# HueCodes/sudoku-vision

Hardware: AMD Instinct MI355X
Metric: end-to-end frames/sec (1080p->81 digits) (higher is better)
Workload: dtype f32

## Files before the change

sudoku-vision_amd/csrc/k1_threshold.hip:

```cpp
#include "sv_device.h"
#include "sv_internal.h"
#include "k2_cells_body.h"

namespace {

constexpr int TW = 64, TH = 32;
constexpr int GW = TW + 14, GH = TH + 14;
constexpr int BW = TW + 10, BH = TH + 10;

struct Taps11 { float k[11]; };

__global__ __launch_bounds__(256) void k_preprocess_any(const u8 *__restrict__ bgr, int H, int W, ptrdiff_t pitch,
                                                          ptrdiff_t img_stride, u8 *__restrict__ out, Taps11 taps)
{
    __shared__ u8 g[GH][GW + 2];
    __shared__ unsigned short hb[GH][BW + 2];
    __shared__ float bl[BH][BW + 1];
    __shared__ float rw[BH][TW + 1];

    const int tid = threadIdx.x;
    const int x0 = blockIdx.x * TW, y0 = blockIdx.y * TH;
    const u8 *img = bgr + (ptrdiff_t)blockIdx.z * img_stride;
    u8 *dst = out + (ptrdiff_t)blockIdx.z * H * W;

    for (int i = tid; i < GH * GW; i += 256) {
        const int ly = i / GW, lx = i - ly * GW;
        const int sx = sv_reflect101(sv_clamp(x0 - 7 + lx, -2, W + 1), W);
        const int sy = sv_reflect101(sv_clamp(y0 - 7 + ly, -2, H + 1), H);
        const u8 *p = img + (ptrdiff_t)sy * pitch + (ptrdiff_t)sx * 3;
        g[ly][lx] = (u8)sv_gray_px(p[0], p[1], p[2]);
    }
    __syncthreads();

    for (int i = tid; i < GH * BW; i += 256) {
        const int ly = i / BW, bq = i - ly * BW;
        const int lc = sv_clamp(x0 - 5 + bq, 0, W - 1) - (x0 - 7);
        hb[ly][bq] = (unsigned short)(16 * (g[ly][lc - 2] + g[ly][lc + 2]) + 64 * (g[ly][lc - 1] + g[ly][lc + 1]) +
                                      96 * g[ly][lc]);
    }
    __syncthreads();

    for (int i = tid; i < BH * BW; i += 256) {
        const int br = i / BW, bq = i - br * BW;
        const int lr = sv_clamp(y0 - 5 + br, 0, H - 1) - (y0 - 7);
        const unsigned v = 16u * (hb[lr - 2][bq] + hb[lr + 2][bq]) + 64u * (hb[lr - 1][bq] + hb[lr + 1][bq]) + 96u * hb[lr][bq];
        bl[br][bq] = (float)((v + 32768u) >> 16);
    }
    __syncthreads();

    for (int i = tid; i < BH * TW; i += 256) {
        const int br = i / TW, x = i - br * TW;
        float acc = __fmul_rn(taps.k[0], bl[br][x]);
#pragma unroll
        for (int j = 1; j < 11; j++) acc = __builtin_fmaf(bl[br][x + j], taps.k[j], acc);
        rw[br][x] = acc;
    }
    __syncthreads();

    for (int i = tid; i < TH * TW; i += 256) {
        const int y = i / TW, x = i - y * TW;
        if (x0 + x >= W || y0 + y >= H) continue;
        float acc = __fmul_rn(taps.k[5], rw[y + 5][x]);
#pragma unroll
        for (int j = 1; j <= 5; j++) acc = __builtin_fmaf(__fadd_rn(rw[y + 5 + j][x], rw[y + 5 - j][x]), taps.k[5 + j], acc);
        const int mean = sv_clamp(__float2int_rn(acc), 0, 255);
        const int src = (int)bl[y + 5][x + 5];
        dst[(ptrdiff_t)(y0 + y) * W + (x0 + x)] = (src - mean <= -2) ? 255 : 0;
    }
}


typedef unsigned int u32;
struct __attribute__((packed, aligned(4))) u32x3 { u32 a, b, c; };
typedef float f32x4_t __attribute__((ext_vector_type(4)));

__device__ __forceinline__ float lane_prev(float v)
{
    return __int_as_float(__builtin_amdgcn_update_dpp(0, __float_as_int(v), 0x138 , 0xf, 0xf, true));
}
__device__ __forceinline__ float lane_next(float v)
{
    return __int_as_float(__builtin_amdgcn_update_dpp(0, __float_as_int(v), 0x130 , 0xf, 0xf, true));
}
__device__ __forceinline__ u32 lane_next_u32(u32 v) { return __float_as_uint(lane_next(__uint_as_float(v))); }
__device__ __forceinline__ float add_prev(float a, float b)
{
    float r;
    asm("v_add_f32_dpp %0, %1, %2 wave_shr:1 row_mask:0xf bank_mask:0xf bound_ctrl:0" : "=v"(r) : "v"(a), "v"(b));
    return r;
}
__device__ __forceinline__ float add_next(float a, float b)
{
    float r;
    asm("v_add_f32_dpp %0, %1, %2 wave_shl:1 row_mask:0xf bank_mask:0xf bound_ctrl:0" : "=v"(r) : "v"(a), "v"(b));
    return r;
}

__device__ __forceinline__ float gray_f32(float b, float g, float r)
{
    return floorf(__builtin_fmaf(b, 3735.f / 32768.f, __builtin_fmaf(g, 19235.f / 32768.f, __builtin_fmaf(r, 9798.f / 32768.f, 0.5f))));
}
__device__ __forceinline__ float blur5(float a, float b, float c, float d, float e)
{
    return __builtin_fmaf(6.f, c, __builtin_fmaf(4.f, b + d, a + e));
}

template <int TW, int TH, int NT, int RC, int RE>
__global__ __launch_bounds__(NT) void k_preprocess_f32(const u8 *__restrict__ bgr, int H, int W, ptrdiff_t pitch,
                                                       ptrdiff_t img_stride, u8 *__restrict__ out, Taps11 taps, int aligned4)
{
    constexpr int GW = TW + 16, GH = TH + 14, BH = TH + 10, NG = GW / 4, NK = TW / 4, NWAVE = NT / 64;
    constexpr int ROWS_PER_WAVE = 64 / NG;
    static_assert(BH * TW <= GH * GW, "rw must fit in hf");
    __shared__ __attribute__((aligned(16))) float smem[GH * GW + BH * GW];
    f32x4_t *hf4 = (f32x4_t *)smem;
    f32x4_t *rw4 = (f32x4_t *)smem;
    f32x4_t *bf4 = (f32x4_t *)(smem + GH * GW);
    float *bf = smem + GH * GW;

    const int tid = threadIdx.x, lane = tid & 63, wave = tid >> 6;
    const int x0 = blockIdx.x * TW, y0 = blockIdx.y * TH;
    const u8 *img = bgr + (ptrdiff_t)blockIdx.z * img_stride;
    u8 *dst = out + (ptrdiff_t)blockIdx.z * H * W;

    {
        const int rl = lane / NG, g = lane - rl * NG;
        const int gx = x0 - 8 + 4 * g;
        const bool fast = aligned4 && gx >= 0 && gx + 3 < W;
        for (int base = 0; base < GH; base += NWAVE * ROWS_PER_WAVE) {
            const int ly = base + wave * ROWS_PER_WAVE + rl;
            const int lyc = ly < GH ? ly : GH - 1;
            const int sy = sv_reflect101(sv_clamp(y0 - 7 + lyc, -2, H + 1), H);
            const u8 *row = img + (ptrdiff_t)sy * pitch;
            float p0, p1, p2, p3;
            if (fast) {
                const u32x3 d = *(const u32x3 *)(row + 3 * gx);
                p0 = gray_f32((float)(d.a & 255), (float)((d.a >> 8) & 255), (float)((d.a >> 16) & 255));
                p1 = gray_f32((float)(d.a >> 24), (float)(d.b & 255), (float)((d.b >> 8) & 255));
                p2 = gray_f32((float)((d.b >> 16) & 255), (float)(d.b >> 24), (float)(d.c & 255));
                p3 = gray_f32((float)((d.c >> 8) & 255), (float)((d.c >> 16) & 255), (float)(d.c >> 24));
            } else {
                float q[4];
                for (int i = 0; i < 4; i++) {
                    const int sx = sv_reflect101(sv_clamp(gx + i, -2, W + 1), W);
                    const u8 *p = row + (ptrdiff_t)sx * 3;
                    q[i] = gray_f32((float)p[0], (float)p[1], (float)p[2]);
                }
                p0 = q[0]; p1 = q[1]; p2 = q[2]; p3 = q[3];
            }
            const float l2 = lane_prev(p2), l3 = lane_prev(p3), r0 = lane_next(p0), r1 = lane_next(p1);
            f32x4_t h;
            h[0] = blur5(l2, l3, p0, p1, p2);
            h[1] = blur5(l3, p0, p1, p2, p3);
            h[2] = blur5(p0, p1, p2, p3, r0);
            h[3] = blur5(p1, p2, p3, r0, r1);
            if (lane < ROWS_PER_WAVE * NG && ly < GH) hf4[ly * NG + g] = h;
        }
    }
    __syncthreads();

    {
        constexpr int NCH = (BH + RC - 1) / RC;
        for (int it = tid; it < NCH * NG; it += NT) {
            const int ch = it / NG, g = it - ch * NG;
            const int br0 = ch * RC;
            f32x4_t win[RC + 4];
#pragma unroll
            for (int r = 0; r < RC + 4; r++) win[r] = hf4[(br0 + r < GH ? br0 + r : GH - 1) * NG + g];
#pragma unroll
            for (int r = 0; r < RC; r++) {
                if (br0 + r < BH) {
                    f32x4_t o;
#pragma unroll
                    for (int c = 0; c < 4; c++)
                        o[c] = floorf(__builtin_fmaf(blur5(win[r][c], win[r + 1][c], win[r + 2][c], win[r + 3][c], win[r + 4][c]), 1.f / 256.f, 0.5f));
                    bf4[(br0 + r) * NG + g] = o;
                }
            }
        }
    }
    __syncthreads();

    if (x0 < 5 || x0 + TW + 5 > W || y0 < 5 || y0 + TH + 5 > H) {
        for (int it = tid; it < BH * GW; it += NT) {
            const int br = it / GW, c = it - br * GW;
            const int q = x0 - 8 + c;
            if (q < 0 || q >= W) {
                const int sc = sv_clamp(q, 0, W - 1) - (x0 - 8);
                if (sc >= 0 && sc < GW) bf[br * GW + c] = bf[br * GW + sc];
            }
        }
        __syncthreads();
        for (int it = tid; it < BH * NG; it += NT) {
            const int br = it / NG, g = it - br * NG;
            const int r = y0 - 5 + br;
            if (r < 0 || r >= H) {
                const int sr = sv_clamp(r, 0, H - 1) - (y0 - 5);
                if (sr >= 0 && sr < BH) bf4[it] = bf4[sr * NG + g];
            }
        }
        __syncthreads();
    }

    for (int it = tid; it < BH * NK; it += NT) {
        const int br = it / NK, k = it - br * NK;
        const f32x4_t *src = bf4 + br * NG + k;
        const f32x4_t a0 = src[0], a1 = src[1], a2 = src[2], a3 = src[3], a4 = src[4];
        const float v[14] = {a0[3], a1[0], a1[1], a1[2], a1[3], a2[0], a2[1], a2[2], a2[3], a3[0], a3[1], a3[2], a3[3], a4[0]};
        f32x4_t o;
#pragma unroll
        for (int c = 0; c < 4; c++) {
            float acc = __fmul_rn(taps.k[0], v[c]);
#pragma unroll
            for (int j = 1; j < 11; j++) acc = __builtin_fmaf(v[c + j], taps.k[j], acc);
            o[c] = acc;
        }
        rw4[it] = o;
    }
    __syncthreads();

    {
        constexpr int NCH = (TH + RE - 1) / RE;
        for (int it = tid; it < NCH * NK; it += NT) {
            const int ch = it / NK, k = it - ch * NK;
            const int yb = ch * RE;
            f32x4_t win[RE + 10];
#pragma unroll
            for (int r = 0; r < RE + 10; r++) win[r] = rw4[(yb + r < BH ? yb + r : BH - 1) * NK + k];
#pragma unroll
            for (int r = 0; r < RE; r++) {
                const int y = yb + r;
                if (y >= TH || y0 + y >= H) continue;
                const f32x4_t srcv = bf4[(y + 5) * NG + k + 2];
                u32 o = 0;
#pragma unroll
                for (int c = 0; c < 4; c++) {
                    float acc = __fmul_rn(taps.k[5], win[r + 5][c]);
#pragma unroll
                    for (int j = 1; j <= 5; j++) acc = __builtin_fmaf(__fadd_rn(win[r + 5 + j][c], win[r + 5 - j][c]), taps.k[5 + j], acc);
                    o |= (__fsub_rn(rintf(acc), srcv[c]) >= 2.f ? 255u : 0u) << (8 * c);
                }
                const int gx = x0 + 4 * k;
                u8 *d = dst + (ptrdiff_t)(y0 + y) * W + gx;
                if (aligned4 && gx + 3 < W) *(u32 *)d = o;
                else
                    for (int c = 0; c < 4; c++)
                        if (gx + c < W) d[c] = (u8)(o >> (8 * c));
            }
        }
    }
}

__device__ __forceinline__ float pick4(const f32x4_t &v, int e) { return e == 0 ? v[0] : e == 1 ? v[1] : e == 2 ? v[2] : v[3]; }

constexpr int MARCH_STRIP = 240;

typedef float f32x2_t __attribute__((ext_vector_type(2)));
struct RowPairs { f32x2_t p[12]; };

__device__ __forceinline__ f32x2_t pkfma(f32x2_t a, f32x2_t b, f32x2_t c) { return __builtin_elementwise_fma(a, b, c); }
__device__ __forceinline__ f32x2_t bc2(float v) { return (f32x2_t){v, v}; }

template <bool BITS>
__device__ __forceinline__ void march_item(const u8 *__restrict__ bgr, int H, int W, ptrdiff_t pitch, ptrdiff_t img_stride, u8 *__restrict__ out,
                                              const Taps11 &taps, const RowPairs &rp, int TH, int nstrips, int nbands, int item, f32x4_t (*sdl)[64])
{
    const int lane = threadIdx.x & 63;
    const int strip = item % nstrips, band = (item / nstrips) % nbands, frame = item / (nstrips * nbands);
    const u8 *img = bgr + (ptrdiff_t)frame * img_stride;
    u8 *dst = out + (ptrdiff_t)frame * H * (BITS ? W >> 3 : W);

    const int xs0 = strip * MARCH_STRIP - 8;
    const int cx0 = xs0 + 4 * lane;
    const int ldx = 3 * sv_clamp(cx0, 0, W - 4);
    const bool edge_l = xs0 < 0, edge_r = xs0 + 256 > W;
    const int yb = band * TH, ye = (yb + TH < H) ? yb + TH : H;
    const int qs = sv_clamp(yb - 5, 0, H - 1);
    const int N = (ye + 4) - qs + 1;
    const int emit_from = yb + 5 - qs;
    const int srcl_hi = (W - 1 - xs0) >> 2;
    const bool store_lane = lane >= 2 && lane < 62 && cx0 < W && (!BITS || ((lane - 2) & 3) == 0);

    auto load_raw = [&](int gy) -> u32x3 { return *(const u32x3 *)(img + (ptrdiff_t)sv_reflect101(gy, H) * pitch + ldx); };
    auto hrow = [&](const u32x3 &d) -> f32x4_t {
        const f32x2_t cb = bc2(3735.f / 32768.f), cg = bc2(19235.f / 32768.f), cr = bc2(9798.f / 32768.f), half = bc2(0.5f);
        const f32x2_t b01 = {(float)(d.a & 255), (float)(d.a >> 24)}, g01 = {(float)((d.a >> 8) & 255), (float)(d.b & 255)},
                      r01 = {(float)((d.a >> 16) & 255), (float)((d.b >> 8) & 255)};
        const f32x2_t b23 = {(float)((d.b >> 16) & 255), (float)((d.c >> 8) & 255)}, g23 = {(float)(d.b >> 24), (float)((d.c >> 16) & 255)},
                      r23 = {(float)(d.c & 255), (float)(d.c >> 24)};
        const f32x2_t y01 = __builtin_elementwise_floor(pkfma(b01, cb, pkfma(g01, cg, pkfma(r01, cr, half))));
        const f32x2_t y23 = __builtin_elementwise_floor(pkfma(b23, cb, pkfma(g23, cg, pkfma(r23, cr, half))));
        float p0 = y01[0], p1 = y01[1], p2 = y23[0], p3 = y23[1];
        if (edge_l) {
            const float n1 = lane_next(p1), n2 = lane_next(p2);
            if (cx0 == -4) { p2 = n2; p3 = n1; }
        }
        if (edge_r) {
            const float q1 = lane_prev(p1), q2 = lane_prev(p2);
            if (cx0 == W) { p0 = q2; p1 = q1; }
        }
        f32x4_t h;
        h[0] = __builtin_fmaf(6.f, p0, __builtin_fmaf(4.f, add_prev(p3, p1), add_prev(p2, p2)));
        h[1] = __builtin_fmaf(6.f, p1, __builtin_fmaf(4.f, p0 + p2, add_prev(p3, p3)));
        h[2] = __builtin_fmaf(6.f, p2, __builtin_fmaf(4.f, p1 + p3, add_next(p0, p0)));
        h[3] = __builtin_fmaf(6.f, p3, __builtin_fmaf(4.f, add_next(p0, p2), add_next(p1, p1)));
        return h;
    };
    auto finish_row = [&](const f32x4_t &a, const f32x4_t &b, const f32x4_t &c, const f32x4_t &d, const f32x4_t &e, f32x4_t &bfv, f32x4_t &rwv) {
        const f32x2_t four = bc2(4.f), six = bc2(6.f), inv = bc2(1.f / 256.f), half = bc2(0.5f);
        const f32x2_t s01 = pkfma(six, c.xy, pkfma(four, b.xy + d.xy, a.xy + e.xy)), s23 = pkfma(six, c.zw, pkfma(four, b.zw + d.zw, a.zw + e.zw));
        const f32x2_t n01 = __builtin_elementwise_floor(pkfma(s01, inv, half)), n23 = __builtin_elementwise_floor(pkfma(s23, inv, half));
        bfv = (f32x4_t){n01[0], n01[1], n23[0], n23[1]};
        if (edge_l) {
            const float v0 = __int_as_float(__builtin_amdgcn_readlane(__float_as_int(bfv[0]), 2));
            if (cx0 < 0) { bfv[0] = v0; bfv[1] = v0; bfv[2] = v0; bfv[3] = v0; }
        }
        if (edge_r) {
            const float v1 = __int_as_float(__builtin_amdgcn_readlane(__float_as_int(bfv[3]), srcl_hi));
            if (cx0 >= W) { bfv[0] = v1; bfv[1] = v1; bfv[2] = v1; bfv[3] = v1; }
        }
        f32x4_t pv, nx;
#pragma unroll
        for (int i = 0; i < 4; i++) { pv[i] = lane_prev(bfv[i]); nx[i] = lane_next(bfv[i]); }
        const float pp3 = lane_prev(pv[3]), nn0 = lane_next(nx[0]);
        const float v[14] = {pp3, pv[0], pv[1], pv[2], pv[3], bfv[0], bfv[1], bfv[2], bfv[3], nx[0], nx[1], nx[2], nx[3], nn0};
        f32x2_t d01 = bc2(v[0]) * rp.p[0], d23 = bc2(v[2]) * rp.p[0];
#pragma unroll
        for (int j = 1; j < 12; j++) {
            d01 = pkfma(bc2(v[j]), rp.p[j], d01);
            d23 = pkfma(bc2(v[2 + j]), rp.p[j], d23);
        }
        rwv = (f32x4_t){d01[0], d01[1], d23[0], d23[1]};
    };

    constexpr int PF = 4, NPH = 12;
    f32x4_t hw[6];
    hw[2] = hrow(load_raw(qs - 2)); hw[3] = hrow(load_raw(qs - 1)); hw[4] = hrow(load_raw(qs)); hw[5] = hrow(load_raw(qs + 1));
    hw[0] = hw[2]; hw[1] = hw[2];
    u32x3 raw[PF];
#pragma unroll
    for (int i = 0; i < PF; i++) raw[i] = load_raw(qs + 2 + i);

    f32x4_t cur_bf = {0.f, 0.f, 0.f, 0.f};
    f32x4_t win[NPH];
#pragma unroll
    for (int k = 0; k < NPH; k++) win[k] = (f32x4_t){0.f, 0.f, 0.f, 0.f};

    for (int base = 0; base < N; base += NPH) {
#pragma unroll
        for (int ph = 0; ph < NPH; ph++) {
            const int i = base + ph;
            if (i < N) {
                const int q = qs + i;
                const u32x3 raw_cur = raw[ph % PF];
                raw[ph % PF] = load_raw(q + 2 + PF < H + 2 ? q + 2 + PF : H + 1);
                if (q <= H - 1) {
                    hw[ph % 6] = hrow(raw_cur);
                    finish_row(hw[(ph + 2) % 6], hw[(ph + 3) % 6], hw[(ph + 4) % 6], hw[(ph + 5) % 6], hw[ph % 6], cur_bf, win[ph]);
                } else {
                    win[ph] = win[(ph + NPH - 1) % NPH];
                }
                if (i == 0) {
#pragma unroll
                    for (int k = 1; k < NPH; k++) win[k] = win[0];
                }
                sdl[i & 7][lane] = cur_bf + 8388610.f;
                if (i >= emit_from) {
                    const int yo = q - 5;
                    const f32x4_t thr = sdl[(i - 5) & 7][lane];
                    const f32x4_t &wc = win[(ph + NPH - 5) % NPH];
                    f32x2_t a01 = bc2(taps.k[5]) * wc.xy, a23 = bc2(taps.k[5]) * wc.zw;
#pragma unroll
                    for (int j = 1; j <= 5; j++) {
                        const f32x4_t &wp = win[(ph + NPH - 5 + j) % NPH], &wm = win[(ph + 2 * NPH - 5 - j) % NPH];
                        a01 = pkfma(wp.xy + wm.xy, bc2(taps.k[5 + j]), a01);
                        a23 = pkfma(wp.zw + wm.zw, bc2(taps.k[5 + j]), a23);
                    }
                    const f32x2_t r01 = a01 + bc2(8388608.f), r23 = a23 + bc2(8388608.f);
                    const float m0 = r01[0], m1 = r01[1], m2 = r23[0], m3 = r23[1];
                    u32 o = 0;
                    asm("v_cmp_ge_f32 vcc, %1, %2\n\tv_addc_co_u32 %0, vcc, %0, %0, vcc" : "+v"(o) : "v"(m3), "v"(thr[3]) : "vcc");
                    asm("v_cmp_ge_f32 vcc, %1, %2\n\tv_addc_co_u32 %0, vcc, %0, %0, vcc" : "+v"(o) : "v"(m2), "v"(thr[2]) : "vcc");
                    asm("v_cmp_ge_f32 vcc, %1, %2\n\tv_addc_co_u32 %0, vcc, %0, %0, vcc" : "+v"(o) : "v"(m1), "v"(thr[1]) : "vcc");
                    asm("v_cmp_ge_f32 vcc, %1, %2\n\tv_addc_co_u32 %0, vcc, %0, %0, vcc" : "+v"(o) : "v"(m0), "v"(thr[0]) : "vcc");
                    if (BITS) {
                        const u32 a = o | (lane_next_u32(o) << 4);
                        const u32 w16 = a | (lane_next_u32(lane_next_u32(a)) << 8);
                        if (store_lane) *(unsigned short *)(dst + (ptrdiff_t)yo * (W >> 3) + (cx0 >> 3)) = (unsigned short)w16;
                    } else if (store_lane) {
                        *(u32 *)(dst + (ptrdiff_t)yo * W + cx0) = ((o * 0x00204081u) & 0x01010101u) * 255u;
                    }
                }
            }
        }
    }
}

template <bool BITS>
__global__ __launch_bounds__(256) void k_preprocess_march(const u8 *__restrict__ bgr, int H, int W, ptrdiff_t pitch, ptrdiff_t img_stride,
                                                             u8 *__restrict__ out, Taps11 taps, RowPairs rp, int TH, int nstrips, int nbands, int nitems)
{
    __shared__ __attribute__((aligned(16))) f32x4_t sdl[4][8][64];
    const int wave = __builtin_amdgcn_readfirstlane(threadIdx.x >> 6);
    const int item = blockIdx.x * 4 + wave;
    if (item >= nitems) return;
    march_item<BITS>(bgr, H, W, pitch, img_stride, out, taps, rp, TH, nstrips, nbands, item, sdl[wave]);
}

__global__ __launch_bounds__(256) void k_preprocess_warp_fused(const u8 *__restrict__ bgr, int n, int H, int W, ptrdiff_t pitch, ptrdiff_t img_stride,
                                                               u8 *__restrict__ out, Taps11 taps, RowPairs rp, int TH, int nstrips, int nbands,
                                                               const double *__restrict__ minv, u8 *__restrict__ cells)
{
    __shared__ __attribute__((aligned(16))) f32x4_t sdl[4][8][64];
    __shared__ sv_k2::CellsLds cl;
    const int items = nstrips * nbands, k1_wgs = (items + 3) / 4, per_frame = k1_wgs + 81;
    const int j = blockIdx.x >> 3, frame = (j / per_frame) * 8 + (blockIdx.x & 7), within = j % per_frame;
    if (frame >= n) return;
    if (within < k1_wgs) {
        const int wave = __builtin_amdgcn_readfirstlane(threadIdx.x >> 6), local = within * 4 + wave;
        if (local < items) march_item<false>(bgr, H, W, pitch, img_stride, out, taps, rp, TH, nstrips, nbands, frame * items + local, sdl[wave]);
    } else {
        sv_k2::warp_cells_item(bgr, H, W, pitch, img_stride, minv, cells, frame, within - k1_wgs, cl);
    }
}

__global__ void k_gray(const u8 *__restrict__ bgr, int H, int W, ptrdiff_t pitch, ptrdiff_t img_stride, u8 *__restrict__ gray)
{
    const int x = blockIdx.x * blockDim.x + threadIdx.x, y = blockIdx.y;
    if (x >= W) return;
    const u8 *p = bgr + (ptrdiff_t)blockIdx.z * img_stride + (ptrdiff_t)y * pitch + (ptrdiff_t)x * 3;
    gray[((ptrdiff_t)blockIdx.z * H + y) * W + x] = (u8)sv_gray_px(p[0], p[1], p[2]);
}

struct FxTaps { int k[7]; int n; };

__global__ void k_blur(const u8 *__restrict__ src, int H, int W, FxTaps t, u8 *__restrict__ dst)
{
    const int x = blockIdx.x * blockDim.x + threadIdx.x, y = blockIdx.y;
    if (x >= W) return;
    const u8 *s = src + (ptrdiff_t)blockIdx.z * H * W;
    const int r = t.n / 2;
    unsigned acc = 0;
    for (int i = 0; i < t.n; i++) {
        const u8 *row = s + (ptrdiff_t)sv_reflect101(y + i - r, H) * W;
        unsigned h = 0;
        for (int j = 0; j < t.n; j++) h += (unsigned)t.k[j] * row[sv_reflect101(x + j - r, W)];
        acc += (unsigned)t.k[i] * h;
    }
    dst[((ptrdiff_t)blockIdx.z * H + y) * W + x] = (u8)((acc + 32768u) >> 16);
}

struct FTaps { float k[31]; int n; };

__device__ __forceinline__ float row_value(const u8 *row, int x, int W, const FTaps &t)
{
    const int r = t.n / 2;
    float acc;
    if (t.n <= 5) {
        acc = __fmul_rn((float)row[x], t.k[r]);
        for (int j = 1; j <= r; j++) {
            const float pr = __fadd_rn((float)row[sv_clamp(x - j, 0, W - 1)], (float)row[sv_clamp(x + j, 0, W - 1)]);
            acc = __builtin_fmaf(pr, t.k[r + j], acc);
        }
    } else {
        acc = __fmul_rn(t.k[0], (float)row[sv_clamp(x - r, 0, W - 1)]);
        for (int j = 1; j < t.n; j++) acc = __builtin_fmaf((float)row[sv_clamp(x + j - r, 0, W - 1)], t.k[j], acc);
    }
    return acc;
}

__global__ void k_adaptive_threshold(const u8 *__restrict__ src, int H, int W, FTaps t, int idelta, int type_inv, u8 *__restrict__ dst)
{
    const int x = blockIdx.x * blockDim.x + threadIdx.x, y = blockIdx.y;
    if (x >= W) return;
    const u8 *s = src + (ptrdiff_t)blockIdx.z * H * W;
    const int r = t.n / 2;
    float acc = __fmul_rn(t.k[r], row_value(s + (ptrdiff_t)y * W, x, W, t));
    for (int j = 1; j <= r; j++) {
        const float lo = row_value(s + (ptrdiff_t)sv_clamp(y + j, 0, H - 1) * W, x, W, t);
        const float hi = row_value(s + (ptrdiff_t)sv_clamp(y - j, 0, H - 1) * W, x, W, t);
        acc = __builtin_fmaf(__fadd_rn(lo, hi), t.k[r + j], acc);
    }
    const int mean = sv_clamp(__float2int_rn(acc), 0, 255);
    const int d = (int)s[(ptrdiff_t)y * W + x] - mean;
    const bool on = type_inv ? (d <= -idelta) : (d > -idelta);
    dst[((ptrdiff_t)blockIdx.z * H + y) * W + x] = on ? 255 : 0;
}

}

static RowPairs row_pairs(const Taps11 &t)
{
    RowPairs rp;
    for (int j = 0; j < 12; j++) rp.p[j] = (f32x2_t){j < 11 ? t.k[j] : 0.f, j > 0 ? t.k[j - 1] : 0.f};
    return rp;
}

static void march_shape(int n, int H, int W, int &nstrips, int &nbands, int &TH)
{
    nstrips = (W + MARCH_STRIP - 1) / MARCH_STRIP;
    nbands = (12288 + n * nstrips - 1) / (n * nstrips);
    if (nbands > H / 32) nbands = H / 32;
    if (nbands < 1) nbands = 1;
    TH = (H + nbands - 1) / nbands;
    nbands = (H + TH - 1) / TH;
}

int svk_preprocess_bits(sv_ctx *ctx, const u8 *bgr, int n, int H, int W, ptrdiff_t pitch, ptrdiff_t img_stride, uint32_t *bits, hipStream_t s)
{
    if (H < 16 || W < 16 || (W & 31) || (pitch % 4) || (img_stride % 4) || ((uintptr_t)bgr % 4))
        return sv_fail(SV_ERR_UNSUPPORTED, "sv_preprocess_bits_u8: needs H, W >= 16, W %% 32 == 0 and a 4-byte aligned frame layout");
    Taps11 t;
    sv_gaussian_taps_f32(11, t.k);
    sv_time_scope ts(ctx, SVK_PREPROCESS, s);
    int nstrips, nbands, TH;
    march_shape(n, H, W, nstrips, nbands, TH);
    const int nitems = n * nstrips * nbands;
    hipLaunchKernelGGL(k_preprocess_march<true>, dim3((nitems + 3) / 4), dim3(256), 0, s, bgr, H, W, pitch, img_stride, (u8 *)bits, t, row_pairs(t), TH, nstrips, nbands, nitems);
    SV_LAUNCH_CHECK("k_preprocess_march<bits>");
    return SV_OK;
}

int svk_preprocess_warp_fused(sv_ctx *ctx, const u8 *bgr, int n, int H, int W, ptrdiff_t pitch, ptrdiff_t img_stride, u8 *binary, const double *minv, u8 *cells,
                              hipStream_t s)
{
    if (H < 16 || W < 16 || (W & 3) || (pitch % 4) || (img_stride % 4) || ((uintptr_t)bgr % 4) || ((uintptr_t)binary % 4))
        return sv_fail(SV_ERR_UNSUPPORTED, "sv_preprocess_warp_cells_u8: needs H, W >= 16, W %% 4 == 0 and a 4-byte aligned layout");
    Taps11 t;
    sv_gaussian_taps_f32(11, t.k);
    sv_time_scope ts(ctx, SVK_FUSED12, s);
    int nstrips, nbands, TH;
    march_shape(n, H, W, nstrips, nbands, TH);
    const long per_frame = (nstrips * nbands + 3) / 4 + 81;
    const long blocks = (long)((n + 7) / 8) * per_frame * 8;
    hipLaunchKernelGGL(k_preprocess_warp_fused, dim3((unsigned)blocks), dim3(256), 0, s, bgr, n, H, W, pitch, img_stride, binary, t, row_pairs(t), TH, nstrips, nbands, minv, cells);
    SV_LAUNCH_CHECK("k_preprocess_warp_fused");
    return SV_OK;
}

int svk_preprocess(sv_ctx *ctx, const u8 *bgr, int n, int H, int W, ptrdiff_t pitch, ptrdiff_t img_stride, u8 *binary, hipStream_t s)
{
    Taps11 t;
    sv_gaussian_taps_f32(11, t.k);
    sv_time_scope ts(ctx, SVK_PREPROCESS, s);
    if (H < 16 || W < 16) {
        dim3 grid((W + TW - 1) / TW, (H + TH - 1) / TH, n);
        hipLaunchKernelGGL(k_preprocess_any, grid, dim3(256), 0, s, bgr, H, W, pitch, img_stride, binary, t);
    } else {
        constexpr int FW = 64, FH = 64;
        const int aligned4 = (pitch % 4 == 0) && (img_stride % 4 == 0) && (W % 4 == 0) && ((uintptr_t)bgr % 4 == 0) && ((uintptr_t)binary % 4 == 0);
        dim3 grid((W + FW - 1) / FW, (H + FH - 1) / FH, n);
        if (aligned4) {
            int nstrips, nbands, TH;
            march_shape(n, H, W, nstrips, nbands, TH);
            const int nitems = n * nstrips * nbands;
            hipLaunchKernelGGL(k_preprocess_march<false>, dim3((nitems + 3) / 4), dim3(256), 0, s, bgr, H, W, pitch, img_stride, binary, t, row_pairs(t), TH, nstrips, nbands, nitems);
        } else {
            hipLaunchKernelGGL((k_preprocess_f32<64, 64, 512, 3, 2>), grid, dim3(512), 0, s, bgr, H, W, pitch, img_stride, binary, t, aligned4);
        }
    }
    SV_LAUNCH_CHECK("k_preprocess");
    return SV_OK;
}

int svk_gray(const u8 *bgr, int n, int H, int W, ptrdiff_t pitch, ptrdiff_t img_stride, u8 *gray, hipStream_t s)
{
    dim3 grid((W + 255) / 256, H, n);
    hipLaunchKernelGGL(k_gray, grid, dim3(256), 0, s, bgr, H, W, pitch, img_stride, gray);
    SV_LAUNCH_CHECK("k_gray");
    return SV_OK;
}

int svk_blur(const u8 *src, int n, int H, int W, int ksize, u8 *dst, hipStream_t s)
{
    static const int tab[4][7] = {{256, 0, 0, 0, 0, 0, 0}, {64, 128, 64, 0, 0, 0, 0}, {16, 64, 96, 64, 16, 0, 0}, {8, 28, 56, 72, 56, 28, 8}};
    FxTaps t;
    t.n = ksize;
    for (int i = 0; i < 7; i++) t.k[i] = tab[ksize / 2][i];
    dim3 grid((W + 255) / 256, H, n);
    hipLaunchKernelGGL(k_blur, grid, dim3(256), 0, s, src, H, W, t, dst);
    SV_LAUNCH_CHECK("k_blur");
    return SV_OK;
}

int svk_adaptive_threshold(const u8 *src, int n, int H, int W, int block, const float *taps, int idelta, int type_inv, u8 *dst, hipStream_t s)
{
    FTaps t;
    t.n = block;
    for (int i = 0; i < 31; i++) t.k[i] = i < block ? taps[i] : 0.f;
    dim3 grid((W + 255) / 256, H, n);
    hipLaunchKernelGGL(k_adaptive_threshold, grid, dim3(256), 0, s, src, H, W, t, idelta, type_inv, dst);
    SV_LAUNCH_CHECK("k_adaptive_threshold");
    return SV_OK;
}
```

Measured before the change: 193,400.

## Compute grayscale and Gaussian blur in packed 16-bit integers via dot4

Replaces the f32 grayscale conversion and 5-tap binomial blur in the marching kernel with integer arithmetic. The grayscale step uses v_dot4_u32_u8 on byte-packed BGR with split low/high coefficient bytes. Each pair of pixels is then packed into one 32-bit register and blurred with packed u16 multiply-adds. The aim is to cut VALU instruction count and the registers needed to hold the row window. The 16-bit sums must stay exactly within range (max 255*256), and the grayscale rounding must still match the reference. Edge-lane handling now relies on new helpers such as lane_next_u32, which are not defined in this diff.

Measured after the change: 190,900. -1.3%, worse.

```diff
diff --git a/sudoku-vision_amd/csrc/k1_threshold.hip b/sudoku-vision_amd/csrc/k1_threshold.hip
--- a/sudoku-vision_amd/csrc/k1_threshold.hip
+++ b/sudoku-vision_amd/csrc/k1_threshold.hip
@@ -261,6 +261,14 @@
 __device__ __forceinline__ f32x2_t pkfma(f32x2_t a, f32x2_t b, f32x2_t c) { return __builtin_elementwise_fma(a, b, c); }
 __device__ __forceinline__ f32x2_t bc2(float v) { return (f32x2_t){v, v}; }
 
+typedef unsigned short u16x2_t __attribute__((ext_vector_type(2)));
+struct HRow { u16x2_t a, b; };
+__device__ __forceinline__ u16x2_t as_u16x2(u32 v) { return __builtin_bit_cast(u16x2_t, v); }
+__device__ __forceinline__ u32 as_u32(u16x2_t v) { return __builtin_bit_cast(u32, v); }
+__device__ __forceinline__ u32 lane_prev_u32(u32 v) { return __float_as_uint(lane_prev(__uint_as_float(v))); }
+__device__ __forceinline__ u16x2_t pkmad4(u16x2_t x, u16x2_t y) { u32 k = 0x00040004u; asm("" : "+s"(k)); return x * as_u16x2(k) + y; }
+__device__ __forceinline__ u16x2_t pkmad6(u16x2_t x, u16x2_t y) { return x * (u16x2_t){6, 6} + y; }
+
 template <bool BITS>
 __device__ __forceinline__ void march_item(const u8 *__restrict__ bgr, int H, int W, ptrdiff_t pitch, ptrdiff_t img_stride, u8 *__restrict__ out,
                                               const Taps11 &taps, const RowPairs &rp, int TH, int nstrips, int nbands, int item, f32x4_t (*sdl)[64])
@@ -282,35 +290,39 @@
     const bool store_lane = lane >= 2 && lane < 62 && cx0 < W && (!BITS || ((lane - 2) & 3) == 0);
 
     auto load_raw = [&](int gy) -> u32x3 { return *(const u32x3 *)(img + (ptrdiff_t)sv_reflect101(gy, H) * pitch + ldx); };
-    auto hrow = [&](const u32x3 &d) -> f32x4_t {
-        const f32x2_t cb = bc2(3735.f / 32768.f), cg = bc2(19235.f / 32768.f), cr = bc2(9798.f / 32768.f), half = bc2(0.5f);
-        const f32x2_t b01 = {(float)(d.a & 255), (float)(d.a >> 24)}, g01 = {(float)((d.a >> 8) & 255), (float)(d.b & 255)},
-                      r01 = {(float)((d.a >> 16) & 255), (float)((d.b >> 8) & 255)};
-        const f32x2_t b23 = {(float)((d.b >> 16) & 255), (float)((d.c >> 8) & 255)}, g23 = {(float)(d.b >> 24), (float)((d.c >> 16) & 255)},
-                      r23 = {(float)(d.c & 255), (float)(d.c >> 24)};
-        const f32x2_t y01 = __builtin_elementwise_floor(pkfma(b01, cb, pkfma(g01, cg, pkfma(r01, cr, half))));
-        const f32x2_t y23 = __builtin_elementwise_floor(pkfma(b23, cb, pkfma(g23, cg, pkfma(r23, cr, half))));
-        float p0 = y01[0], p1 = y01[1], p2 = y23[0], p3 = y23[1];
+    auto hrow = [&](const u32x3 &d) -> HRow {
+        constexpr u32 LO = 46u | 70u << 8 | 140u << 16, HI = 29u | 150u << 8 | 76u << 16;
+        const u32 px1 = __builtin_amdgcn_alignbyte(d.b, d.a, 3), px2 = __builtin_amdgcn_alignbyte(d.c, d.b, 2);
+        u32 p01, p23, t0, t1, t2, t3, u0, u1, u2, u3;
+        asm("v_dot4_u32_u8 %2, %10, %14, %18\n\tv_dot4_u32_u8 %6, %10, %15, 0\n\t"
+            "v_dot4_u32_u8 %3, %11, %14, %18\n\tv_dot4_u32_u8 %7, %11, %15, 0\n\t"
+            "v_dot4_u32_u8 %4, %12, %14, %18\n\tv_dot4_u32_u8 %8, %12, %15, 0\n\t"
+            "v_dot4_u32_u8 %5, %13, %16, %18\n\tv_dot4_u32_u8 %9, %13, %17, 0\n\t"
+            "v_lshl_add_u32 %2, %6, 8, %2\n\tv_lshl_add_u32 %3, %7, 8, %3\n\tv_lshl_add_u32 %4, %8, 8, %4\n\tv_lshl_add_u32 %5, %9, 8, %5\n\t"
+            "v_perm_b32 %0, %3, %2, %19\n\tv_perm_b32 %1, %5, %4, %19"
+            : "=&v"(p01), "=&v"(p23), "=&v"(t0), "=&v"(t1), "=&v"(t2), "=&v"(t3), "=&v"(u0), "=&v"(u1), "=&v"(u2), "=&v"(u3)
+            : "v"(d.a), "v"(px1), "v"(px2), "v"(d.c), "s"(LO), "s"(HI), "s"(LO << 8), "s"(HI << 8), "v"(32768u), "s"(0x0c060c02u));
         if (edge_l) {
-            const float n1 = lane_next(p1), n2 = lane_next(p2);
-            if (cx0 == -4) { p2 = n2; p3 = n1; }
+            const u32 n01 = lane_next_u32(p01), n23 = lane_next_u32(p23);
+            if (cx0 == -4) p23 = (n23 & 0xffffu) | (n01 & 0xffff0000u);
         }
         if (edge_r) {
-            const float q1 = lane_prev(p1), q2 = lane_prev(p2);
-            if (cx0 == W) { p0 = q2; p1 = q1; }
-        }
-        f32x4_t h;
-        h[0] = __builtin_fmaf(6.f, p0, __builtin_fmaf(4.f, add_prev(p3, p1), add_prev(p2, p2)));
-        h[1] = __builtin_fmaf(6.f, p1, __builtin_fmaf(4.f, p0 + p2, add_prev(p3, p3)));
-        h[2] = __builtin_fmaf(6.f, p2, __builtin_fmaf(4.f, p1 + p3, add_next(p0, p0)));
-        h[3] = __builtin_fmaf(6.f, p3, __builtin_fmaf(4.f, add_next(p0, p2), add_next(p1, p1)));
+            const u32 q01 = lane_prev_u32(p01), q23 = lane_prev_u32(p23);
+            if (cx0 == W) p01 = (q23 & 0xffffu) | (q01 & 0xffff0000u);
+        }
+        const u32 l23 = lane_prev_u32(p23), nx01 = lane_next_u32(p01);
+        const u16x2_t lp = as_u16x2(__builtin_amdgcn_alignbit(p01, l23, 16));
+        const u16x2_t pp = as_u16x2(__builtin_amdgcn_alignbit(p23, p01, 16));
+        const u16x2_t pr = as_u16x2(__builtin_amdgcn_alignbit(nx01, p23, 16));
+        HRow h;
+        h.a = pkmad6(as_u16x2(p01), pkmad4(lp + pp, as_u16x2(l23) + as_u16x2(p23)));
+        h.b = pkmad6(as_u16x2(p23), pkmad4(pp + pr, as_u16x2(p01) + as_u16x2(nx01)));
         return h;
     };
-    auto finish_row = [&](const f32x4_t &a, const f32x4_t &b, const f32x4_t &c, const f32x4_t &d, const f32x4_t &e, f32x4_t &bfv, f32x4_t &rwv) {
-        const f32x2_t four = bc2(4.f), six = bc2(6.f), inv = bc2(1.f / 256.f), half = bc2(0.5f);
-        const f32x2_t s01 = pkfma(six, c.xy, pkfma(four, b.xy + d.xy, a.xy + e.xy)), s23 = pkfma(six, c.zw, pkfma(four, b.zw + d.zw, a.zw + e.zw));
-        const f32x2_t n01 = __builtin_elementwise_floor(pkfma(s01, inv, half)), n23 = __builtin_elementwise_floor(pkfma(s23, inv, half));
-        bfv = (f32x4_t){n01[0], n01[1], n23[0], n23[1]};
+    auto finish_row = [&](const HRow &a, const HRow &b, const HRow &c, const HRow &d, const HRow &e, f32x4_t &bfv, f32x4_t &rwv) {
+        const u16x2_t rnd = {128, 128};
+        const u32 s01 = as_u32(pkmad6(c.a, pkmad4(b.a + d.a, a.a + e.a)) + rnd), s23 = as_u32(pkmad6(c.b, pkmad4(b.b + d.b, a.b + e.b)) + rnd);
+        bfv = (f32x4_t){(float)((s01 >> 8) & 255), (float)(s01 >> 24), (float)((s23 >> 8) & 255), (float)(s23 >> 24)};
         if (edge_l) {
             const float v0 = __int_as_float(__builtin_amdgcn_readlane(__float_as_int(bfv[0]), 2));
             if (cx0 < 0) { bfv[0] = v0; bfv[1] = v0; bfv[2] = v0; bfv[3] = v0; }
@@ -334,7 +346,7 @@
     };
 
     constexpr int PF = 4, NPH = 12;
-    f32x4_t hw[6];
+    HRow hw[6];
     hw[2] = hrow(load_raw(qs - 2)); hw[3] = hrow(load_raw(qs - 1)); hw[4] = hrow(load_raw(qs)); hw[5] = hrow(load_raw(qs + 1));
     hw[0] = hw[2]; hw[1] = hw[2];
     u32x3 raw[PF];
```
